# automl/TransformersCanDoBayesianInference

Measured on AMD Instinct MI355X. Metric: synthetic datasets/sec (GP prior, bptt=2000), higher is better.
Workload: dtype fp16; 1 GPU; priors.fast_gp, bptt=2000, num_features=18, emsize=512, nhead=4, nhid=1024, nlayers=6, 1000 bars (BASELINE.json configs[1]); per_gpu_batch=64, global_batch=64, aggregate_k_gradients=1, aggregate_streams=0, aggregate_stacked=False, seq_len=2000, parallelism=dp1, micro_batch_streams=2, eval_pos=weighted sampler(2000)

## Files before the change

transformerscandobayesianinference_amd/csrc/gemm_tn.hip:

```cpp
#include <type_traits>
#include "pfn_device.h"
#include "pfn_kernels.h"

namespace pfn {

PFN_DEV int xcd_remap(int bid, int nwg) {
  const int q = nwg >> 3, r = nwg & 7, xcd = bid & 7;
  return (xcd < r ? xcd * (q + 1) : r * (q + 1) + (xcd - r) * q) + (bid >> 3);
}
typedef __attribute__((address_space(1))) const void gvoid_t;
typedef __attribute__((address_space(3))) void lvoid_t;

constexpr int TN_BMK = 32;

template <typename T>
__global__ __launch_bounds__(256, 2) void gemm_tn_kernel(GemmTN g) {
  constexpr int RB = 128 * sizeof(T);
  constexpr int TILE = TN_BMK * RB;
  extern __shared__ __attribute__((aligned(16))) char smem_raw[];
  LdsPtr smem = lds_cast(smem_raw);
  auto tileA = [&](int buf) { return smem + buf * 2 * TILE; };
  auto tileB = [&](int buf) { return smem + buf * 2 * TILE + TILE; };

  const int p0 = blockIdx.y * 128, q0 = blockIdx.x * 128;
// ... 30 lines not shown
      if constexpr (sizeof(T) == 2) {
        const X8<T> v = __builtin_bit_cast(X8<T>, sa.regs[i]);
#pragma unroll
        for (int e = 0; e < 8; ++e) csum[e] += (float)v[e];
      } else {
        const f32x4 v = __builtin_bit_cast(f32x4, sa.regs[i]);
#pragma unroll
        for (int e = 0; e < 4; ++e) csum[e] += v[e];
      }
    }
  };
  sa.issue(A, g.lda, rows_total, colsA);
  sb.issue(B, g.ldb, rows_total, colsB);
  add_colsum();
  sa.template commit<true>(tileA(0));
  sb.template commit<true>(tileB(0));
  __syncthreads();
  for (int t = 0; t < nt; ++t) {
    const int cur = t & 1;
    if (t + 1 < nt) {
      const long r1 = (long)(t + 1) * TN_BMK;
      sa.issue(A + r1 * g.lda, g.lda, rows_total - (int)r1, colsA);
      sb.issue(B + r1 * g.ldb, g.ldb, rows_total - (int)r1, colsB);
      add_colsum();
    }
    const lds_char* ta = tileA(cur);
    const lds_char* tb = tileB(cur);
#pragma unroll
    for (int ks = 0; ks < TN_BMK; ks += 16) {
      Frag<T> fa[2], fb[2];
#pragma unroll
      for (int i = 0; i < 2; ++i) fa[i] = load_frag_tr<T, RB, 1>(ta, ks, wp * 64 + i * 32);
#pragma unroll
      for (int j = 0; j < 2; ++j) fb[j] = load_frag_tr<T, RB, 1>(tb, ks, wq * 64 + j * 32);
#pragma unroll
      for (int i = 0; i < 2; ++i)
#pragma unroll
        for (int j = 0; j < 2; ++j) acc[i][j] = mma32(fa[i], fb[j], acc[i][j]);
    }
    if (t + 1 < nt) {
      sa.template commit<true>(tileA(cur ^ 1));
      sb.template commit<true>(tileB(cur ^ 1));
    }
    __syncthreads();
  }

  const float osc = loss_scale_down(g.scale_amax);
  if (do_colsum) {
    constexpr int NCH = RB / 16;
    float* red = reinterpret_cast<float*>(smem_raw);
#pragma unroll
    for (int e = 0; e < EPC; ++e) red[threadIdx.x * EPC + e] = csum[e];
    __syncthreads();
    if (threadIdx.x < NCH) {
#pragma unroll
      for (int e = 0; e < EPC; ++e) {
        float t = 0.f;
        for (int j = 0; j < 256 / NCH; ++j) t += red[(j * NCH + threadIdx.x) * EPC + e];
        const int col = p0 + threadIdx.x * EPC + e;
        if (col < g.P) unsafeAtomicAdd(g.colsum + col, t * loss_scale_down(g.scale_amax));
      }
    }
  }
#pragma unroll
  for (int i = 0; i < 2; ++i)
#pragma unroll
    for (int j = 0; j < 2; ++j)
#pragma unroll
      for (int r = 0; r < 16; ++r) {
        const int p = p0 + wp * 64 + i * 32 + acc_row(r, lane);
        const int q = q0 + wq * 64 + j * 32 + (lane & 31);
        if (p < g.P && q < g.Q) {
          float* c = g.C + (long)p * g.ldc + q;
          if (g.atomic) unsafeAtomicAdd(c, acc[i][j][r] * osc);
          else *c = acc[i][j][r] * osc;
        }
      }
}

#ifndef PFN_TNB_KT
#define PFN_TNB_KT 64
#define PFN_TNB_NS 2
#endif
constexpr int TNB_KT = PFN_TNB_KT;
constexpr int TNB_NS = PFN_TNB_NS;
constexpr int TNB_TILE = TNB_KT * 512;
constexpr int TNB_PW = TNB_KT / 16;
constexpr int TNB_LDS = TNB_NS * 2 * TNB_TILE;
static_assert(TNB_LDS <= 160 * 1024 && TNB_KT % 16 == 0 && TNB_NS >= 2 && (TNB_NS - 2) * 2 * TNB_PW < 64, "weight-gradient ring does not fit");

template <typename T>
__global__ __launch_bounds__(512, 1) void gemm_tn_big_kernel(GemmTNGroup g) {
  extern __shared__ __attribute__((aligned(16))) char smem_raw[];
  LdsPtr smem = lds_cast(smem_raw);

  const int ntiles = g.tile_start[g.n];
  const int id = xcd_remap(blockIdx.x, ntiles * g.splits);
  const int split = id / ntiles, tile = id % ntiles;
  int pi = 0;
  while (tile >= g.tile_start[pi + 1]) ++pi;
  const TnProblem& pr = g.p[pi];
  const int tq = pr.Q / 256;
  const int tl = tile - g.tile_start[pi];
  const int p0 = (tl / tq) * 256, q0 = (tl % tq) * 256;
  const long mbeg = (long)split * g.m_chunk;
  const long mend = min((long)g.M, mbeg + g.m_chunk);
  const int rows_total = (int)(mend - mbeg);
  if (rows_total <= 0) return;

  const int wave = __builtin_amdgcn_readfirstlane(threadIdx.x >> 6), lane = threadIdx.x & 63;
  const int wp = wave >> 2, wq = wave & 3;

  const T* pa[TNB_PW];
  const T* pb[TNB_PW];
  int prow[TNB_PW];
#pragma unroll
  for (int i = 0; i < TNB_PW; ++i) {
    const int row = (wave + 8 * i) * 2 + (lane >> 5);
    const int unit = ((lane & 31) >> 2) ^ (row & 3);
    const int col = unit * 32 + (lane & 3) * 8;
    prow[i] = row;
    pa[i] = reinterpret_cast<const T*>(pr.A) + mbeg * pr.lda + p0 + col;
    pb[i] = reinterpret_cast<const T*>(pr.B) + mbeg * pr.ldb + q0 + col;
  }
  auto stage = [&](int slot, int r0) {
    LdsPtr ta = smem + slot * 2 * TNB_TILE + wave * 1024;
    LdsPtr tb = ta + TNB_TILE;
#pragma unroll
    for (int i = 0; i < TNB_PW; ++i) {
      const long r = min(r0 + prow[i], rows_total - 1) & g.debug_mask;
      dma16_global(pa[i] + r * pr.lda, ta + i * 8192);
      dma16_global(pb[i] + r * pr.ldb, tb + i * 8192);
    }
  };

  f32x16 acc[4][2];
#pragma unroll
  for (int i = 0; i < 4; ++i)
#pragma unroll
    for (int j = 0; j < 2; ++j)
#pragma unroll
      for (int r = 0; r < 16; ++r) acc[i][j][r] = 0.f;
  f32x16 cs;
#pragma unroll
  for (int r = 0; r < 16; ++r) cs[r] = 0.f;
  const bool do_colsum = pr.colsum != nullptr && q0 == 0;
  Frag<T> ones;
#pragma unroll
  for (int e = 0; e < 8; ++e) ones.v[e] = (T)1.0f;

  const int nt = (rows_total + TNB_KT - 1) / TNB_KT;
#pragma unroll
  for (int st = 0; st < TNB_NS - 1; ++st)
    if (st < nt) stage(st, st * TNB_KT);
  auto wait_stage = [&](int younger) {
    switch (younger) {
      case 0: wait_vm_barrier<0>(); break;
      case 1: wait_vm_barrier<(TNB_NS > 2 ? 1 : 0) * 2 * TNB_PW>(); break;
      case 2: wait_vm_barrier<(TNB_NS > 3 ? 2 : 0) * 2 * TNB_PW>(); break;
      case 3: wait_vm_barrier<(TNB_NS > 4 ? 3 : 0) * 2 * TNB_PW>(); break;
      default: wait_vm_barrier<(TNB_NS - 2) * 2 * TNB_PW>(); break;
    }
  };
  static_assert(TNB_NS <= 6, "wait_stage cases");
  auto main_loop = [&](auto with_colsum) {
    constexpr bool CS = decltype(with_colsum)::value;
    int slot = 0, slot_next = TNB_NS - 1;
    for (int t = 0; t < nt; ++t) {
      wait_stage(min(nt - t - 1, TNB_NS - 2));
      if (t + TNB_NS - 1 < nt) stage(slot_next, (t + TNB_NS - 1) * TNB_KT);
      LdsPtr ta = smem + slot * 2 * TNB_TILE;
      LdsPtr tb = ta + TNB_TILE;
      const int valid = rows_total - t * TNB_KT;
      if (valid < TNB_KT) {
        for (int idx = threadIdx.x; idx < (TNB_KT - valid) * 32; idx += 512) {
          const u32x4 z = {0u, 0u, 0u, 0u};
          lds_write16(ta + (valid + idx / 32) * 512 + (idx % 32) * 16, z);
        }
        __syncthreads();
      }
#pragma unroll
      for (int ks = 0; ks < TNB_KT; ks += 16) {
        Frag<T> fa[4], fb[2];
#pragma unroll
        for (int j = 0; j < 2; ++j) fb[j] = load_frag_tr<T, 512, 1>(tb, ks, wq * 64 + j * 32);
#pragma unroll
        for (int i = 0; i < 4; ++i) fa[i] = load_frag_tr<T, 512, 1>(ta, ks, wp * 128 + i * 32);
#pragma unroll
        for (int i = 0; i < 4; ++i)
#pragma unroll
          for (int j = 0; j < 2; ++j) acc[i][j] = mma32(fa[i], fb[j], acc[i][j]);
        if constexpr (CS) cs = mma32(load_frag_tr<T, 512, 1>(ta, ks, wp * 128 + wq * 32), ones, cs);
      }
      slot_next = slot;
      slot = slot + 1 == TNB_NS ? 0 : slot + 1;
    }
  };
  if (do_colsum) main_loop(std::true_type{});
  else main_loop(std::false_type{});

  const int pv = pr.Pv > 0 ? pr.Pv : pr.P;
  const float osc = loss_scale_down(g.scale_amax);
  if (do_colsum && (lane & 31) == 0) {
#pragma unroll
    for (int r = 0; r < 16; ++r) {
      const int pp = p0 + wp * 128 + wq * 32 + acc_row(r, lane);
      if (pp < pv) unsafeAtomicAdd(pr.colsum + pp, cs[r] * osc);
    }
  }
  const bool atomic = true;
#pragma unroll
  for (int i = 0; i < 4; ++i)
#pragma unroll
    for (int j = 0; j < 2; ++j)
#pragma unroll
      for (int r = 0; r < 16; ++r) {
        const int pp = p0 + wp * 128 + i * 32 + acc_row(r, lane);
        const int qq = q0 + wq * 64 + j * 32 + (lane & 31);
        float* c = pr.C + (long)pp * pr.ldc + qq;
        if (pp >= pv) continue;
        if (atomic) unsafeAtomicAdd(c, acc[i][j][r] * osc);
        else *c += acc[i][j][r] * osc;
      }
}

constexpr int TNW_NW = 4;
constexpr int TNW_PW = TNB_KT / 2 / TNW_NW;
static_assert(TNB_KT == 64 && TNB_NS == 2, "gemm_tn_wide_kernel is written for two 64-token stages");
template <typename T>
__global__ __launch_bounds__(TNW_NW * 64, 1) void gemm_tn_wide_kernel(GemmTNGroup g) {
  extern __shared__ __attribute__((aligned(16))) char smem_raw[];
  LdsPtr smem = lds_cast(smem_raw);
  const int ntiles = g.tile_start[g.n];
  const int id = xcd_remap(blockIdx.x, ntiles * g.splits);
  const int split = id / ntiles, tile = id % ntiles;
  int pi = 0;
  while (tile >= g.tile_start[pi + 1]) ++pi;
  const TnProblem& pr = g.p[pi];
  const int tq = pr.Q / 256;
  const int tl = tile - g.tile_start[pi];
  const int p0 = (tl / tq) * 256, q0 = (tl % tq) * 256;
  const long mbeg = (long)split * g.m_chunk;
  const long mend = min((long)g.M, mbeg + g.m_chunk);
  const int rows_total = (int)(mend - mbeg);
  if (rows_total <= 0) return;
  const int wave = __builtin_amdgcn_readfirstlane(threadIdx.x >> 6), lane = threadIdx.x & 63;
  const int wp = wave >> 1, wq = wave & 1;

  const int prow0 = wave * 2 + (lane >> 5);
  const int pcol = ((((lane & 31) >> 2) ^ (prow0 & 3)) * 32) + (lane & 3) * 8;
  const T* pa = reinterpret_cast<const T*>(pr.A) + mbeg * pr.lda + p0 + pcol;
  const T* pb = reinterpret_cast<const T*>(pr.B) + mbeg * pr.ldb + q0 + pcol;
  const long lda = pr.lda, ldb = pr.ldb;
  auto stage = [&](int slot, int r0) {
    LdsPtr ta = smem + slot * 2 * TNB_TILE + wave * 1024;
    LdsPtr tb = ta + TNB_TILE;
#pragma unroll
    for (int i = 0; i < TNW_PW; ++i) {
      const long r = min(r0 + prow0 + 2 * TNW_NW * i, rows_total - 1) & g.debug_mask;
      dma16_global(pa + r * lda, ta + i * TNW_NW * 1024);
      dma16_global(pb + r * ldb, tb + i * TNW_NW * 1024);
    }
  };

  f32x16 acc[4][4];
#pragma unroll
  for (int i = 0; i < 4; ++i)
#pragma unroll
    for (int j = 0; j < 4; ++j)
#pragma unroll
      for (int r = 0; r < 16; ++r) acc[i][j][r] = 0.f;
  float cs[2] = {0.f, 0.f};
  const bool do_colsum = pr.colsum != nullptr && q0 == 0;

  const int nt = (rows_total + TNB_KT - 1) / TNB_KT;
  struct Frs { Frag<T> a[4], b[4]; };
  auto main_loop = [&](auto with_colsum) {
    constexpr bool CS = decltype(with_colsum)::value;
    Frs f0, f1;
    auto ld = [&](Frs& f, const lds_char* ta, const lds_char* tb, int ks) {
#pragma unroll
      for (int j = 0; j < 4; ++j) f.b[j] = load_frag_tr<T, 512, 1>(tb, ks, wq * 128 + j * 32);
#pragma unroll
      for (int i = 0; i < 4; ++i) f.a[i] = load_frag_tr<T, 512, 1>(ta, ks, wp * 128 + i * 32);
    };
    auto mm = [&](const Frs& f) {
#pragma unroll
      for (int i = 0; i < 4; ++i)
#pragma unroll
        for (int j = 0; j < 4; ++j) acc[i][j] = mma32(f.a[i], f.b[j], acc[i][j]);
      if constexpr (CS) {
#pragma unroll
        for (int c = 0; c < 2; ++c)
#pragma unroll
          for (int e = 0; e < 8; ++e) cs[c] += (float)(wq ? f.a[2 + c] : f.a[c]).v[e];
      }
    };
    auto enter_stage = [&](int t, int slot) {
      wait_vm_barrier<0>();
      if (t + 1 < nt) stage(slot ^ 1, (t + 1) * TNB_KT);
      const int valid = rows_total - t * TNB_KT;
      if (valid < TNB_KT) {
        LdsPtr ta = smem + slot * 2 * TNB_TILE;
        for (int idx = threadIdx.x; idx < (TNB_KT - valid) * 32; idx += TNW_NW * 64) {
          const u32x4 z = {0u, 0u, 0u, 0u};
          lds_write16(ta + (valid + idx / 32) * 512 + (idx % 32) * 16, z);
        }
        __syncthreads();
      }
    };
    int slot = 0;
    enter_stage(0, slot);
    ld(f0, smem, smem + TNB_TILE, 0);
    for (int t = 0; t < nt; ++t) {
      const lds_char* ta = smem + slot * 2 * TNB_TILE;
      const lds_char* tb = ta + TNB_TILE;
      ld(f1, ta, tb, 16);
      PFN_PIN_LDS_MFMA();
      mm(f0);
      PFN_PIN_LDS_MFMA();
      ld(f0, ta, tb, 32);
      PFN_PIN_LDS_MFMA();
      mm(f1);
      PFN_PIN_LDS_MFMA();
      ld(f1, ta, tb, 48);
      PFN_PIN_LDS_MFMA();
      mm(f0);
      PFN_PIN_LDS_MFMA();
      slot ^= 1;
      if (t + 1 < nt) {
        enter_stage(t + 1, slot);
        const lds_char* tan = smem + slot * 2 * TNB_TILE;
        ld(f0, tan, tan + TNB_TILE, 0);
      }
      PFN_PIN_LDS_MFMA();
      mm(f1);
      PFN_PIN_LDS_MFMA();
    }
  };
  stage(0, 0);
  if (do_colsum) main_loop(std::true_type{});
  else main_loop(std::false_type{});

  const int pv = pr.Pv > 0 ? pr.Pv : pr.P;
  const float osc = loss_scale_down(g.scale_amax);
  if (do_colsum) {
#pragma unroll
    for (int c = 0; c < 2; ++c) {
      const float s = cs[c] + __shfl_xor(cs[c], 32, 64);
      const int pp = p0 + wp * 128 + (2 * wq + c) * 32 + (lane & 31);
      if (lane < 32 && pp < pv) unsafeAtomicAdd(pr.colsum + pp, s * osc);
    }
  }
#pragma unroll
  for (int i = 0; i < 4; ++i)
#pragma unroll
    for (int j = 0; j < 4; ++j)
#pragma unroll
      for (int r = 0; r < 16; ++r) {
        const int pp = p0 + wp * 128 + i * 32 + acc_row(r, lane);
        const int qq = q0 + wq * 128 + j * 32 + (lane & 31);
        if (pp < pv) unsafeAtomicAdd(pr.C + (long)pp * pr.ldc + qq, acc[i][j][r] * osc);
      }
}

static bool aligned16(const void* p) { return (reinterpret_cast<uintptr_t>(p) & 15) == 0; }

static int g_tn_debug_wrap = 0;
void set_gemm_tn_debug_wrap(int rows) { g_tn_debug_wrap = rows; }
static int g_tn_group_splits = 0;
void set_gemm_tn_group_splits(int splits) { g_tn_group_splits = splits; }
static bool g_tn_wide = false;
void set_gemm_tn_group_waves(int waves) { g_tn_wide = waves == 4; }

int launch_gemm_tn(GemmTN g, int precision, hipStream_t stream) {
  if (g.M <= 0 || g.P <= 0 || g.Q <= 0) return PFN_OK;
  const size_t es = prec_esize(precision);
  if ((g.lda * es) % 16 || (g.ldb * es) % 16 || !aligned16(g.A) || !aligned16(g.B)) return PFN_ERR_ALIGNMENT;
  const int tp = (g.P + 127) / 128, tq = (g.Q + 127) / 128;
  int splits = (1024 + tp * tq - 1) / (tp * tq);
  const int max_splits = (g.M + 4 * TN_BMK - 1) / (4 * TN_BMK);
  if (splits > max_splits) splits = max_splits;
  if (g.max_splits > 0 && splits > g.max_splits) splits = g.max_splits;
  if (splits < 1) splits = 1;
  if (!g.atomic) splits = 1;
  int chunk = (g.M + splits - 1) / splits;
  chunk = (chunk + TN_BMK - 1) / TN_BMK * TN_BMK;
  splits = (g.M + chunk - 1) / chunk;
  g.m_chunk = chunk;
  const size_t lds = 4 * TN_BMK * 128 * es;
  PFN_DISPATCH_OP(precision, hipLaunchKernelGGL(gemm_tn_kernel<T>, dim3(tq, tp, splits), dim3(256), lds, stream, g));
  return hipGetLastError() == hipSuccess ? PFN_OK : PFN_ERR_LAUNCH;
}

bool gemm_tn_group_supported(const TnProblem& p) {
  return p.P % 256 == 0 && p.Q % 256 == 0 && (p.lda * 2) % 16 == 0 && (p.ldb * 2) % 16 == 0 && aligned16(p.A) && aligned16(p.B);
}

int launch_gemm_tn_group(GemmTNGroup g, int precision, hipStream_t stream) {
  if (g.n <= 0 || g.M <= 0) return PFN_OK;
  if (g.n > TN_GROUP_MAX) return PFN_ERR_ARGUMENT;
  if (!prec_is16(precision)) return PFN_ERR_UNSUPPORTED;
  int tiles = 0;
  for (int i = 0; i < g.n; ++i) {
    if (!gemm_tn_group_supported(g.p[i])) return PFN_ERR_UNSUPPORTED;
    g.tile_start[i] = tiles;
    tiles += (g.p[i].P / 256) * (g.p[i].Q / 256);
  }
  g.tile_start[g.n] = tiles;
  int splits = g.splits;
  if (splits <= 0 && g_tn_group_splits > 0) splits = g_tn_group_splits;
  if (splits <= 0) {
    splits = 8;
    for (int sp = 1; sp <= 8; ++sp) {
      const int blocks = tiles * sp, rounds = (blocks + 255) / 256;
      if (blocks >= 0.9 * rounds * 256) { splits = sp; break; }
    }
  }
  const int max_splits = (g.M + 4 * TNB_KT - 1) / (4 * TNB_KT);
  if (splits > max_splits) splits = max_splits;
  int chunk = (g.M + splits - 1) / splits;
  chunk = (chunk + TNB_KT - 1) / TNB_KT * TNB_KT;
  splits = (g.M + chunk - 1) / chunk;
  g.splits = splits;
  g.m_chunk = chunk;
  g.debug_mask = g_tn_debug_wrap > 0 ? g_tn_debug_wrap - 1 : 0x7fffffff;
  if (g_tn_wide) {
    static LdsAllowance allow_w[2];
    if (precision == PFN_PREC_FP16) {
      allow_w[1].ensure(gemm_tn_wide_kernel<f16>, TNB_LDS);
      hipLaunchKernelGGL(gemm_tn_wide_kernel<f16>, dim3(tiles * splits), dim3(TNW_NW * 64), TNB_LDS, stream, g);
    } else {
      allow_w[0].ensure(gemm_tn_wide_kernel<bf16>, TNB_LDS);
      hipLaunchKernelGGL(gemm_tn_wide_kernel<bf16>, dim3(tiles * splits), dim3(TNW_NW * 64), TNB_LDS, stream, g);
    }
    return hipGetLastError() == hipSuccess ? PFN_OK : PFN_ERR_LAUNCH;
  }
  static LdsAllowance allowance[2];
  if (precision == PFN_PREC_FP16) {
    allowance[1].ensure(gemm_tn_big_kernel<f16>, TNB_LDS);
    hipLaunchKernelGGL(gemm_tn_big_kernel<f16>, dim3(tiles * splits), dim3(512), TNB_LDS, stream, g);
  } else {
    allowance[0].ensure(gemm_tn_big_kernel<bf16>, TNB_LDS);
    hipLaunchKernelGGL(gemm_tn_big_kernel<bf16>, dim3(tiles * splits), dim3(512), TNB_LDS, stream, g);
  }
  return hipGetLastError() == hipSuccess ? PFN_OK : PFN_ERR_LAUNCH;
}

}
```

transformerscandobayesianinference_amd/csrc/pfn_api.hip:

```cpp
#include <algorithm>
#include <cstdarg>
#include <cstdio>
#include <cstring>
#include <mutex>
#include <vector>
#include "pfn_kernels.h"

using namespace pfn;

namespace pfn {
namespace {
struct ProfPair { hipEvent_t a, b; };
std::mutex g_prof_mu;
std::vector<ProfPair> g_prof[PFN_PROF_SLOTS];
std::atomic<int> g_prof_on{0};
}
bool prof_enabled() { return g_prof_on.load(std::memory_order_relaxed) != 0; }
void* prof_begin(int slot, hipStream_t s) {
  const int on = g_prof_on.load(std::memory_order_relaxed);
  if (!on || slot < 0 || slot >= PFN_PROF_SLOTS) return nullptr;
  if (on >= 2 && (slot & ~1) != on - 2) return nullptr;
  ProfPair* p = new ProfPair;
  if (hipEventCreate(&p->a) != hipSuccess || hipEventCreate(&p->b) != hipSuccess) { delete p; return nullptr; }
  (void)hipEventRecord(p->a, s);
// ... 300 lines not shown
  const pfn_model_desc& d = *m.d;
  const int prec = d.precision, E = d.emsize, F = d.nhid;
  const float* params = m.params;
  hipStream_t s = m.s;
  const bool y16u = pl.y16u;
  if (pl.fuse_ln) {
    ProfScope ps(PFN_PROF_GEMM_OUT_LN + prof, s);
    GemmLN g; memset(&g, 0, sizeof(g));
    g.A = u.ctx; g.lda = E; g.B = W(m, p.w_o); g.ldb = E; g.M = rows; g.N = E; g.K = E; g.bias = params + p.b_o;
    set_resid(g, res);
    g.gamma = params + p.g1; g.beta = params + p.be1; g.eps = d.ln_eps;
    g.y = u.y1; g.mean = u.mean1; g.rstd = u.rstd1; g.x_t = u.x1_t; g.y16 = pl.y16;
    PFN_TRY(launch_gemm_ln(g, prec, s));
    res = Resid{nullptr, u.y1, u.mean1, u.rstd1, params + p.g1, params + p.be1};
  } else {
    {
      GemmNT g = nt(u.ctx, E, W(m, p.w_o), E, rows, E, E, EPI_BIAS | (pdrop > 0.f ? 0 : EPI_RESID) | EPI_OUT_F32);
      g.bias = params + p.b_o; g.resid = u.xin; g.ld_resid = E; g.out_f32 = u.y1; g.ld_out_f32 = E;
      if (y16u) { g.flags = EPI_BIAS | EPI_RESID_T | EPI_OUT_T; g.aux = u.xin_t; g.ld_aux = E; g.out_t = u.y1; g.ld_out_t = E; }
      PFN_TRY(launch_gemm_nt(g, prec, s));
      if (pdrop > 0.f) PFN_TRY(launch_dropout_add(u.y1, u.xin, rows, E, seed[1], pdrop, s));
    }
    PFN_TRY(launch_layernorm_fwd(u.y1, params + p.g1, params + p.be1, y16u ? nullptr : u.x1, u.x1_t, u.mean1, u.rstd1, rows, E, d.ln_eps, prec, s, y16u));
  }
  {
    ProfScope ps(PFN_PROF_GEMM_LIN1 + prof, s);
    GemmNT g = nt(u.x1_t, E, W(m, p.w1), E, rows, F, E, EPI_BIAS | EPI_GELU | EPI_OUT_T | EPI_OUT2_T);
    g.bias = params + p.b1; g.out_t = u.h; g.ld_out_t = F; g.out2_t = u.hpre; g.ld_out2 = F;
    PFN_TRY(launch_gemm_nt(g, prec, s));
    if (pdrop > 0.f) PFN_TRY(launch_dropout_scale(u.h, u.h, u.hpre, u.hpre, rows, F, seed[2], pdrop, prec, s));
  }
  if (pl.fuse_ln) {
    ProfScope ps(PFN_PROF_GEMM_LIN2_LN + prof, s);
    GemmLN g; memset(&g, 0, sizeof(g));
    g.A = u.h; g.lda = F; g.B = W(m, p.w2); g.ldb = F; g.M = rows; g.N = E; g.K = F; g.bias = params + p.b2;
    set_resid(g, res);
    g.gamma = params + p.g2; g.beta = params + p.be2; g.eps = d.ln_eps;
    g.y = u.y2; g.mean = u.mean2; g.rstd = u.rstd2; g.x_t = u.x2_t; g.y16 = pl.y16;
    g.x_f32 = last ? u.x2 : nullptr;
    PFN_TRY(launch_gemm_ln(g, prec, s));
    res = Resid{nullptr, u.y2, u.mean2, u.rstd2, params + p.g2, params + p.be2};
  } else {
    {
      GemmNT g = nt(u.h, F, W(m, p.w2), F, rows, E, F, EPI_BIAS | (pdrop > 0.f ? 0 : EPI_RESID) | EPI_OUT_F32);
      g.bias = params + p.b2; g.resid = u.x1; g.ld_resid = E; g.out_f32 = u.y2; g.ld_out_f32 = E;
      if (y16u) { g.flags = EPI_BIAS | EPI_RESID_T | EPI_OUT_T; g.aux = u.x1_t; g.ld_aux = E; g.out_t = u.y2; g.ld_out_t = E; }
      PFN_TRY(launch_gemm_nt(g, prec, s));
      if (pdrop > 0.f) PFN_TRY(launch_dropout_add(u.y2, u.x1, rows, E, seed[3], pdrop, s));
    }
    PFN_TRY(launch_layernorm_fwd(u.y2, params + p.g2, params + p.be2, (y16u && !last) ? nullptr : u.x2, u.x2_t, u.mean2, u.rstd2, rows, E, d.ln_eps, prec, s, y16u));
  }
  return PFN_OK;
}

int decoder_forward(const Model& m, const void* xt_t, char* dt, char* dpre, float* logits, int rows) {
  const int prec = m.d->precision, E = m.d->emsize, F = m.d->nhid, O = m.d->n_out;
  {
    GemmNT g = nt(xt_t, E, W(m, m.L->dec0_w), E, rows, F, E, EPI_BIAS | EPI_GELU | EPI_OUT_T | EPI_OUT2_T);
    g.bias = m.params + m.L->dec0_b; g.out_t = dt; g.ld_out_t = F; g.out2_t = dpre; g.ld_out2 = F;
    PFN_TRY(launch_gemm_nt(g, prec, m.s));
  }
  GemmNT g = nt(dt, F, W(m, m.L->dec2_w), F, rows, O, F, EPI_BIAS | EPI_OUT_F32);
  g.bias = m.params + m.L->dec2_b; g.out_f32 = logits; g.ld_out_f32 = O;
  return launch_gemm_nt(g, prec, m.s);
}
int decoder_backward_data(const Model& m, const void* dlog_t, const void* dpre, char* dd_t, float* dxt, int rows) {
  const int prec = m.d->precision, E = m.d->emsize, F = m.d->nhid, O = m.d->n_out, npad = m.L->n_out_pad;
  {
    GemmNT g = nt(dlog_t, npad, WT(m, m.L->dec2_wt), npad, rows, F, npad % 64 == 0 ? npad : O, EPI_GELU_BWD | EPI_OUT_T);
    g.aux = dpre; g.ld_aux = F; g.out_t = dd_t; g.ld_out_t = F;
    PFN_TRY(launch_gemm_nt(g, prec, m.s));
  }
  GemmNT g = nt(dd_t, F, WT(m, m.L->dec0_wt), F, rows, E, F, EPI_OUT_F32);
  g.out_f32 = dxt; g.ld_out_f32 = E;
  return launch_gemm_nt(g, prec, m.s);
}

bool tn_set_groupable(const std::vector<TnProblem>& probs, int prec) {
  bool grouped = prec_is16(prec);
  for (const TnProblem& t : probs) grouped = grouped && gemm_tn_group_supported(t);
  return grouped;
}
int launch_tn_set(const std::vector<TnProblem>& probs, int rows, int prec, bool det, const float* lsc, int prof_slot, hipStream_t s, bool allow_group = true) {
  if (!(allow_group && tn_set_groupable(probs, prec))) {
    for (const TnProblem& t : probs) {
      GemmTN g = tn(t.A, t.lda, t.B, t.ldb, t.C, t.ldc, rows, t.Pv ? t.Pv : t.P, t.Q, t.colsum);
      if (det) g.max_splits = 1;
      g.scale_amax = lsc;
      PFN_TRY(launch_gemm_tn(g, prec, s));
    }
    return PFN_OK;
  }
  for (size_t i0 = 0; i0 < probs.size(); i0 += TN_GROUP_MAX) {
    ProfScope ps(prof_slot, s);
    GemmTNGroup g;
    memset(&g, 0, sizeof(g));
    g.n = (int)std::min<size_t>(TN_GROUP_MAX, probs.size() - i0);
    g.M = rows;
    g.splits = det ? 1 : 0;
    g.scale_amax = lsc;
    for (int i = 0; i < g.n; ++i) g.p[i] = probs[i0 + i];
    PFN_TRY(launch_gemm_tn_group(g, prec, s));
  }
  return PFN_OK;
}

struct LnSinks { float *dgamma, *dbeta, *dbias; };
struct LayerGrads {
  const void* dout; int dout_is_t;
  const void* y2; const float *mean2, *rstd2, *gamma2; const void* y1; const float *mean1, *rstd1, *gamma1; const void* hpre;
  char *dy2_t, *dy2m_t, *dh_t, *dy1_t, *dqkv_t, *dx1_t;
  LnSinks ln2, ln1;
  float* ln_part;
};
GemmLNB lnb(const Model& m, const Plan& pl, const float* lsc, const void* A, long lda, const void* Bw, long ldb, int K, const void* aux, const void* y,
            const float* mean, const float* rstd, const float* gamma, void* dx_t, const LnSinks& sink, int rows) {
  GemmLNB g; memset(&g, 0, sizeof(g));
  g.A = A; g.lda = lda; g.B = Bw; g.ldb = ldb; g.M = rows; g.N = m.d->emsize; g.K = K; g.aux = aux;
  g.y = y; g.mean = mean; g.rstd = rstd; g.gamma = gamma; g.dx_t = dx_t; g.dgamma = sink.dgamma; g.dbeta = sink.dbeta; g.scale_amax = lsc; g.y16 = pl.y16_any;
  return g;
}
GemmLNB lnb_dy1(const Model& m, const Plan& pl, const float* lsc, const LayerP& t, const LayerGrads& g, int rows) {
  const int F = m.d->nhid;
  return lnb(m, pl, lsc, g.dh_t, F, WT(m, t.w1), F, F, g.dy2_t, g.y1, g.mean1, g.rstd1, g.gamma1, g.dy1_t, g.ln1, rows);
}
GemmLNB lnb_dx(const Model& m, const Plan& pl, const float* lsc, const LayerP& t, const char* dqkv_t, const char* dy1_t, const LayerGrads& below, int rows) {
  const int E = m.d->emsize;
  return lnb(m, pl, lsc, dqkv_t, 3 * E, WT(m, t.w_in), 3 * E, 3 * E, dy1_t, below.y2, below.mean2, below.rstd2, below.gamma2, below.dy2_t, below.ln2, rows);
}
bool lnbwd_fusable(const Model& m, const Plan& pl, const float* lsc, const LayerGrads& g0, int rows) {
  const LayerP& t = m.L->layer_t[0];
  return pl.lnb_eligible && gemm_lnbwd_supported(lnb_dy1(m, pl, lsc, t, g0, rows)) && gemm_lnbwd_supported(lnb_dx(m, pl, lsc, t, g0.dqkv_t, g0.dy1_t, g0, rows));
}
int layer_backward_to_dy1(const Model& m, const LayerP& t, const LayerGrads& g, int rows, const Plan& pl, bool fuse_lnb, bool ln2_done, const float* lsc,
                          float pdrop, unsigned seed2, int prof) {
  const int prec = m.d->precision, E = m.d->emsize, F = m.d->nhid;
  hipStream_t s = m.s;
  if (!ln2_done)
    PFN_TRY(launch_layernorm_bwd(g.dout, g.dout_is_t, g.y2, g.gamma2, g.mean2, g.rstd2, nullptr, g.dy2_t, g.ln2.dgamma, g.ln2.dbeta, g.ln2.dbias, rows, E, prec, s,
                                 g.ln_part, lsc, pl.y16_any));
  const char* dy2_op = g.dy2_t;
  if (pdrop > 0.f) { PFN_TRY(launch_dropout_scale(g.dy2_t, g.dy2m_t, nullptr, nullptr, rows, E, seed2, pdrop, prec, s)); dy2_op = g.dy2m_t; }
  {
    ProfScope ps(PFN_PROF_GEMM_DHPRE + prof, s);
    GemmNT gm = nt(dy2_op, E, WT(m, t.w2), E, rows, F, E, EPI_GELU_BWD | EPI_OUT_T);
    gm.aux = g.hpre; gm.ld_aux = F; gm.out_t = g.dh_t; gm.ld_out_t = F;
    PFN_TRY(launch_gemm_nt(gm, prec, s));
  }
  if (fuse_lnb) {
    ProfScope ps(PFN_PROF_GEMM_DY1 + prof, s);
    PFN_TRY(launch_gemm_lnbwd(lnb_dy1(m, pl, lsc, t, g, rows), prec, s));
  } else {
    {
      GemmNT gm = nt(g.dh_t, F, WT(m, t.w1), F, rows, E, F, EPI_RESID_T | EPI_OUT_T);
      gm.aux = g.dy2_t; gm.ld_aux = E; gm.out_t = g.dx1_t; gm.ld_out_t = E;
      PFN_TRY(launch_gemm_nt(gm, prec, s));
    }
    PFN_TRY(launch_layernorm_bwd(g.dx1_t, 1, g.y1, g.gamma1, g.mean1, g.rstd1, nullptr, g.dy1_t, g.ln1.dgamma, g.ln1.dbeta, g.ln1.dbias, rows, E, prec, s,
                                 g.ln_part, lsc, pl.y16_any));
  }
  return PFN_OK;
}
int layer_backward_dx(const Model& m, const LayerP& t, const char* dqkv_t, const char* dy1_t, int rows, const Plan& pl, const float* lsc, const LayerGrads* below,
                      float* gA, char* gA_t, bool out_f32, int prof) {
  const int prec = m.d->precision, E = m.d->emsize;
  if (below) {
    ProfScope ps(PFN_PROF_GEMM_DX + prof, m.s);
    return launch_gemm_lnbwd(lnb_dx(m, pl, lsc, t, dqkv_t, dy1_t, *below, rows), prec, m.s);
  }
  GemmNT g = nt(dqkv_t, 3 * E, WT(m, t.w_in), 3 * E, rows, E, 3 * E, EPI_RESID_T | (out_f32 ? EPI_OUT_F32 : EPI_OUT_T));
  g.aux = dy1_t; g.ld_aux = E; g.out_f32 = gA; g.ld_out_f32 = E; g.out_t = gA_t; g.ld_out_t = E;
  return launch_gemm_nt(g, prec, m.s);
}

}

extern "C" {

static bool g_gp_planes = true;
static bool g_fuse_delta = true;
static int g_default_schedule = 0;
static bool top_layer_on_test_rows(const pfn_model_desc& d, int S, int sep, float pdrop) {
  return !(d.schedule & PFN_SCHED_TOP_LAYER_ALL_ROWS) && d.nlayers > 0 && pdrop == 0.f && d.dropout == 0.f && sep < S && 4L * sep >= S;
}
static bool top_layer_on_test_rows_ragged(const pfn_model_desc& d, int S, const Ragged& rg, float pdrop) {
// ... 1028 lines not shown
```

transformerscandobayesianinference_amd/csrc/pfn_device.h:

```cpp
#pragma once
#include <hip/hip_runtime.h>
#include <stdint.h>

namespace pfn {

typedef __bf16 bf16;
typedef __attribute__((ext_vector_type(8))) __bf16 bf16x8;
typedef __attribute__((ext_vector_type(4))) __bf16 bf16x4;
typedef __attribute__((ext_vector_type(2))) __bf16 bf16x2;
typedef _Float16 f16;
typedef __attribute__((ext_vector_type(8))) _Float16 f16x8;
typedef __attribute__((ext_vector_type(4))) _Float16 f16x4;
typedef __attribute__((ext_vector_type(2))) _Float16 f16x2;
typedef __attribute__((ext_vector_type(16))) float f32x16;
typedef __attribute__((ext_vector_type(4))) float f32x4;
typedef __attribute__((ext_vector_type(2))) float f32x2;
typedef __attribute__((ext_vector_type(4))) unsigned int u32x4;
typedef __attribute__((ext_vector_type(2))) unsigned int u32x2;
template <typename T> struct OpVec;
template <> struct OpVec<bf16> { typedef bf16x8 x8; typedef bf16x4 x4; typedef bf16x2 x2; };
template <> struct OpVec<f16> { typedef f16x8 x8; typedef f16x4 x4; typedef f16x2 x2; };
template <> struct OpVec<float> { typedef f32x4 x8; typedef f32x4 x4; typedef f32x2 x2; };
template <typename T> using X8 = typename OpVec<T>::x8;
template <typename T> using X4 = typename OpVec<T>::x4;
// ... 151 lines not shown
    const int colb = (col0 + 16 * g + 4 * (i & 3)) * 2;
    const int ra = (MAP == 1) ? (k0 + 8 * h) : (k0 + 4 * h);
    const int rb = (MAP == 1) ? (k0 + 8 * h + 4) : (k0 + 8 + 4 * h);
    const auto lo = ds_read_tr16_b64<T>(tile + (ra + (i >> 2)) * STRIDE + colb);
    const auto hi = ds_read_tr16_b64<T>(tile + (rb + (i >> 2)) * STRIDE + colb);
    f.v = __builtin_shufflevector(lo, hi, 0, 1, 2, 3, 4, 5, 6, 7);
  } else {
    const int colb = (col0 + (l & 31)) * 4;
#pragma unroll
    for (int e = 0; e < 8; ++e) {
      const int row = (MAP == 1) ? (k0 + 8 * h + e) : (k0 + 8 * (e >> 2) + 4 * h + (e & 3));
      f.v[e] = lds_read_f32(tile + row * STRIDE + colb);
    }
  }
  return f;
}

template <typename T> PFN_DEV void store_row_block(T* row_block, const float (&v)[16], int h, bool valid) {
  if constexpr (sizeof(T) == 2) {
#pragma unroll
    for (int p = 0; p < 2; ++p) {
      typedef typename OpVec<T>::x2 x2;
      x2 a0 = {(T)v[8 * p + 0], (T)v[8 * p + 1]}, a1 = {(T)v[8 * p + 2], (T)v[8 * p + 3]};
      x2 b0 = {(T)v[8 * p + 4], (T)v[8 * p + 5]}, b1 = {(T)v[8 * p + 6], (T)v[8 * p + 7]};
      const auto r0 = __builtin_amdgcn_permlane32_swap(__builtin_bit_cast(unsigned, a0), __builtin_bit_cast(unsigned, b0), false, false);
      const auto r1 = __builtin_amdgcn_permlane32_swap(__builtin_bit_cast(unsigned, a1), __builtin_bit_cast(unsigned, b1), false, false);
      const u32x4 w = {r0[0], r1[0], r0[1], r1[1]};
      if (valid) *reinterpret_cast<u32x4*>(row_block + 16 * p + 8 * h) = w;
    }
  } else {
#pragma unroll
    for (int rg = 0; rg < 4; ++rg)
      if (valid) *reinterpret_cast<f32x4*>(row_block + 8 * rg + 4 * h) = f32x4{v[4 * rg], v[4 * rg + 1], v[4 * rg + 2], v[4 * rg + 3]};
  }
}

template <typename T> PFN_DEV void store_frag_pair_blocked(T* block, const Frag<T>& f0, const Frag<T>& f1, int j, int h, bool valid) {
  char* base = reinterpret_cast<char*>(block);
  if constexpr (sizeof(T) == 2) {
#pragma unroll
    for (int p = 0; p < 2; ++p) {
      const u32x4 d = __builtin_bit_cast(u32x4, p == 0 ? f0.v : f1.v);
      const auto r0 = __builtin_amdgcn_permlane32_swap(d[0], d[2], false, false);
      const auto r1 = __builtin_amdgcn_permlane32_swap(d[1], d[3], false, false);
      const u32x4 w = {r0[0], r1[0], r0[1], r1[1]};
      if (valid) __builtin_nontemporal_store(w, reinterpret_cast<u32x4*>(base + ((p * 32 + j) * 2 + h) * 16));
    }
  } else {
#pragma unroll
    for (int p = 0; p < 2; ++p) {
      const Frag<T>& f = p == 0 ? f0 : f1;
#pragma unroll
      for (int sub = 0; sub < 2; ++sub)
        if (valid) __builtin_nontemporal_store(f32x4{f.v[4 * sub], f.v[4 * sub + 1], f.v[4 * sub + 2], f.v[4 * sub + 3]},
                                               reinterpret_cast<f32x4*>(base + (((2 * p + sub) * 32 + j) * 2 + h) * 16));
    }
  }
}
template <typename T> PFN_DEV int blocked_chunk_row(int w) { return (w >> 1) & 31; }
template <typename T> PFN_DEV int blocked_chunk_col(int w) {
  if constexpr (sizeof(T) == 2) return 16 * (w >> 6) + 8 * (w & 1);
  else return 8 * (w >> 6) + 4 * (w & 1);
}

typedef __amdgpu_buffer_rsrc_t BufRsrc;
PFN_DEV BufRsrc make_rsrc(const void* base, long bytes) {
  const int n = bytes > 0x7ffffff0L ? 0x7ffffff0 : (bytes < 0 ? 0 : (int)bytes);
  return __builtin_amdgcn_make_buffer_rsrc(const_cast<void*>(base), 0, n, 0x00020000);
}
PFN_DEV u32x4 buf_load16(BufRsrc r, int byte_offset) { return __builtin_amdgcn_raw_buffer_load_b128(r, byte_offset, 0, 0); }
constexpr int BUF_OOB = 0x7ffffff0;

struct DmaRsrc { u32x4 w; };
PFN_DEV DmaRsrc make_dma_rsrc(const void* base, long bytes) {
  const unsigned long long p = (unsigned long long)base;
  const int n = bytes > 0x7ffffff0L ? 0x7ffffff0 : (bytes < 0 ? 0 : (int)bytes);
  DmaRsrc r;
  r.w[0] = __builtin_amdgcn_readfirstlane((unsigned)p);
  r.w[1] = __builtin_amdgcn_readfirstlane((unsigned)(p >> 32) & 0xffffu);
  r.w[2] = __builtin_amdgcn_readfirstlane((unsigned)n);
  r.w[3] = 0x00020000u;
  return r;
}
PFN_DEV void dma16(const DmaRsrc& r, LdsPtr lds_dst_uniform, int byte_offset) {
  unsigned keep;
  const unsigned dst = __builtin_amdgcn_readfirstlane((unsigned)(unsigned long long)lds_dst_uniform);
  const u32x4 w = {(unsigned)__builtin_amdgcn_readfirstlane(r.w[0]), (unsigned)__builtin_amdgcn_readfirstlane(r.w[1]),
                   (unsigned)__builtin_amdgcn_readfirstlane(r.w[2]), (unsigned)__builtin_amdgcn_readfirstlane(r.w[3])};
  asm volatile("s_mov_b32 %0, m0\n\ts_mov_b32 m0, %1\n\ts_nop 0\n\tbuffer_load_dwordx4 %2, %3, 0 offen lds\n\ts_mov_b32 m0, %0"
               : "=&s"(keep) : "s"(dst), "v"(byte_offset), "s"(w) : "memory");
}
PFN_DEV void dma4(const DmaRsrc& r, LdsPtr lds_dst_uniform, int byte_offset) {
  unsigned keep;
  const unsigned dst = __builtin_amdgcn_readfirstlane((unsigned)(unsigned long long)lds_dst_uniform);
  const u32x4 w = {(unsigned)__builtin_amdgcn_readfirstlane(r.w[0]), (unsigned)__builtin_amdgcn_readfirstlane(r.w[1]),
                   (unsigned)__builtin_amdgcn_readfirstlane(r.w[2]), (unsigned)__builtin_amdgcn_readfirstlane(r.w[3])};
  asm volatile("s_mov_b32 %0, m0\n\ts_mov_b32 m0, %1\n\ts_nop 0\n\tbuffer_load_dword %2, %3, 0 offen lds\n\ts_mov_b32 m0, %0"
               : "=&s"(keep) : "s"(dst), "v"(byte_offset), "s"(w) : "memory");
}
PFN_DEV void dma16_global(const void* src, LdsPtr lds_dst_uniform) {
  unsigned keep;
  const unsigned dst = __builtin_amdgcn_readfirstlane((unsigned)(unsigned long long)lds_dst_uniform);
  asm volatile("s_mov_b32 %0, m0\n\ts_mov_b32 m0, %1\n\ts_nop 0\n\tglobal_load_lds_dwordx4 %2, off\n\ts_mov_b32 m0, %0"
               : "=&s"(keep) : "s"(dst), "v"(src) : "memory");
}
template <int N> PFN_DEV void wait_vm_barrier() {
  __builtin_amdgcn_s_waitcnt(0x0070 | (N & 15) | ((N >> 4) << 14));
  asm volatile("s_waitcnt vmcnt(%0) lgkmcnt(0)\n\ts_barrier" :: "n"(N) : "memory");
}
PFN_DEV void dma_wait_all() {
  __builtin_amdgcn_s_waitcnt(0x0F70);
  asm volatile("s_waitcnt vmcnt(0)" ::: "memory");
}

template <typename T, int ROWS, int RB, int NT> struct TileStageBuf {
  static constexpr int NCH = RB / 16;
  static constexpr int TOTAL = ROWS * NCH;
  static constexpr int PER = (TOTAL + NT - 1) / NT;
  u32x4 regs[PER];
  int voff[PER];
  PFN_DEV void init(int ld_bytes) {
#pragma unroll
    for (int i = 0; i < PER; ++i) {
      const int id = threadIdx.x + i * NT;
      voff[i] = (TOTAL % NT == 0 || id < TOTAL) ? (id / NCH) * ld_bytes + (id % NCH) * 16 : BUF_OOB;
    }
  }
  PFN_DEV void issue(BufRsrc r, int tile_byte_offset) {
#pragma unroll
    for (int i = 0; i < PER; ++i) regs[i] = buf_load16(r, voff[i] + tile_byte_offset);
  }
  template <int STRIDE> PFN_DEV void commit_p(LdsPtr tile) const {
#pragma unroll
    for (int i = 0; i < PER; ++i) {
      const int id = threadIdx.x + i * NT;
      if (TOTAL % NT != 0 && id >= TOTAL) break;
      lds_write16(tile + (id / NCH) * STRIDE + (id % NCH) * 16, regs[i]);
    }
  }
};

template <typename T, int ROWS, int RB, int NT> struct TileStage {
  static constexpr int NCH = RB / 16;
  static constexpr int TOTAL = ROWS * NCH;
  static constexpr int PER = (TOTAL + NT - 1) / NT;
  static constexpr int EPC = 16 / sizeof(T);
  u32x4 regs[PER];

  PFN_DEV void issue(const T* src, long ld, int rows_valid, int cols_valid) {
#pragma unroll
    for (int i = 0; i < PER; ++i) {
      const int id = threadIdx.x + i * NT;
      const int row = id / NCH, c = id % NCH;
      u32x4 v = {0u, 0u, 0u, 0u};
      if ((TOTAL % NT == 0 || id < TOTAL) && row < rows_valid && (c + 1) * EPC <= cols_valid)
        v = *reinterpret_cast<const u32x4*>(src + (long)row * ld + c * EPC);
      else if ((TOTAL % NT == 0 || id < TOTAL) && row < rows_valid && c * EPC < cols_valid) {
        T tmp[EPC];
#pragma unroll
        for (int e = 0; e < EPC; ++e) tmp[e] = (c * EPC + e < cols_valid) ? src[(long)row * ld + c * EPC + e] : (T)0.f;
        v = *reinterpret_cast<u32x4*>(tmp);
      }
      regs[i] = v;
    }
  }
  template <int STRIDE> PFN_DEV void commit_p(LdsPtr tile) const {
// ... 103 lines not shown
```

Measured before the change: 2513 datasets/s.

## Stage weight-gradient GEMM tiles via buffer-resource DMA with late issue after first MFMA

Replaces per-row global-pointer DMA staging in the TN weight-gradient kernels with a buffer-resource stager that advances a base address per K tile. Out-of-range rows are now zero-filled by the hardware bounds check, so the LDS zero-fill pass and its extra barrier go away. In the big kernel the next stage's loads are issued after the first MFMA sub-step instead of before compute, so address math and issue overlap with matrix work. The cost is a host-side support check with a per-problem fallback when strides or split sizes exceed the buffer range, and the simple two-stage wait assumes the default ring depth.

After: 2548 datasets/s (median of 6 runs). +1.4%, better.

```diff
diff --git a/transformerscandobayesianinference_amd/csrc/gemm_tn.hip b/transformerscandobayesianinference_amd/csrc/gemm_tn.hip
--- a/transformerscandobayesianinference_amd/csrc/gemm_tn.hip
+++ b/transformerscandobayesianinference_amd/csrc/gemm_tn.hip
@@ -136,12 +136,54 @@
 #define PFN_TNB_KT 64
 #define PFN_TNB_NS 2
 #endif
+#ifndef PFN_TNB_LATE_ISSUE
+#define PFN_TNB_LATE_ISSUE 1
+#endif
 constexpr int TNB_KT = PFN_TNB_KT;
 constexpr int TNB_NS = PFN_TNB_NS;
 constexpr int TNB_TILE = TNB_KT * 512;
 constexpr int TNB_PW = TNB_KT / 16;
 constexpr int TNB_LDS = TNB_NS * 2 * TNB_TILE;
 static_assert(TNB_LDS <= 160 * 1024 && TNB_KT % 16 == 0 && TNB_NS >= 2 && (TNB_NS - 2) * 2 * TNB_PW < 64, "weight-gradient ring does not fit");
+constexpr long TN_GROUP_MAX_SPLIT_BYTES = 0x7ffffff0L;
+
+template <int NW> struct TnStager {
+  static constexpr int NP = TNB_KT / 2 / NW;
+  DmaRsrc ra, rb;
+  unsigned a_lo, a_hi, b_lo, b_hi;
+  unsigned step_a, step_b;
+  int va[NP], vb[NP];
+  int wave, srow, mask;
+  PFN_DEV void init(const TnProblem& pr, long mbeg, int rows, int p0, int q0, int wave_, int lane, int debug_mask) {
+    const long lda2 = pr.lda * 2, ldb2 = pr.ldb * 2;
+    ra = make_dma_rsrc(reinterpret_cast<const char*>(pr.A) + mbeg * lda2 + p0 * 2, (rows - 1) * lda2 + 512);
+    rb = make_dma_rsrc(reinterpret_cast<const char*>(pr.B) + mbeg * ldb2 + q0 * 2, (rows - 1) * ldb2 + 512);
+    a_lo = ra.w[0]; a_hi = ra.w[1]; b_lo = rb.w[0]; b_hi = rb.w[1];
+    step_a = __builtin_amdgcn_readfirstlane((unsigned)(TNB_KT * lda2));
+    step_b = __builtin_amdgcn_readfirstlane((unsigned)(TNB_KT * ldb2));
+    wave = wave_; srow = 0; mask = debug_mask;
+    const int row0 = wave * 2 + (lane >> 5);
+    const int colb = ((((lane & 31) >> 2) ^ (row0 & 3)) * 32 + (lane & 3) * 8) * 2;
+#pragma unroll
+    for (int i = 0; i < NP; ++i) {
+      va[i] = (row0 + 2 * NW * i) * (int)lda2 + colb;
+      vb[i] = (row0 + 2 * NW * i) * (int)ldb2 + colb;
+    }
+  }
+  PFN_DEV void issue(LdsPtr slot) {
+    LdsPtr ta = slot + wave * 1024;
+    LdsPtr tb = ta + TNB_TILE;
+#pragma unroll
+    for (int i = 0; i < NP; ++i) {
+      dma16(ra, ta + i * NW * 1024, va[i]);
+      dma16(rb, tb + i * NW * 1024, vb[i]);
+    }
+    dma_rsrc_advance(ra, step_a);
+    dma_rsrc_advance(rb, step_b);
+    srow += TNB_KT;
+    if ((srow & mask) == 0) { ra.w[0] = a_lo; ra.w[1] = a_hi; rb.w[0] = b_lo; rb.w[1] = b_hi; }
+  }
+};
 
 template <typename T>
 __global__ __launch_bounds__(512, 1) void gemm_tn_big_kernel(GemmTNGroup g) {
@@ -165,28 +207,9 @@
   const int wave = __builtin_amdgcn_readfirstlane(threadIdx.x >> 6), lane = threadIdx.x & 63;
   const int wp = wave >> 2, wq = wave & 3;
 
-  const T* pa[TNB_PW];
-  const T* pb[TNB_PW];
-  int prow[TNB_PW];
-#pragma unroll
-  for (int i = 0; i < TNB_PW; ++i) {
-    const int row = (wave + 8 * i) * 2 + (lane >> 5);
-    const int unit = ((lane & 31) >> 2) ^ (row & 3);
-    const int col = unit * 32 + (lane & 3) * 8;
-    prow[i] = row;
-    pa[i] = reinterpret_cast<const T*>(pr.A) + mbeg * pr.lda + p0 + col;
-    pb[i] = reinterpret_cast<const T*>(pr.B) + mbeg * pr.ldb + q0 + col;
-  }
-  auto stage = [&](int slot, int r0) {
-    LdsPtr ta = smem + slot * 2 * TNB_TILE + wave * 1024;
-    LdsPtr tb = ta + TNB_TILE;
-#pragma unroll
-    for (int i = 0; i < TNB_PW; ++i) {
-      const long r = min(r0 + prow[i], rows_total - 1) & g.debug_mask;
-      dma16_global(pa[i] + r * pr.lda, ta + i * 8192);
-      dma16_global(pb[i] + r * pr.ldb, tb + i * 8192);
-    }
-  };
+  TnStager<8> stg;
+  stg.init(pr, mbeg, rows_total, p0, q0, wave, lane, g.debug_mask);
+  static_assert(TnStager<8>::NP == TNB_PW, "wait_stage counts 2 TNB_PW DMA instructions per stage");
 
   f32x16 acc[4][2];
 #pragma unroll
@@ -206,8 +229,9 @@
   const int nt = (rows_total + TNB_KT - 1) / TNB_KT;
 #pragma unroll
   for (int st = 0; st < TNB_NS - 1; ++st)
-    if (st < nt) stage(st, st * TNB_KT);
+    if (st < nt) stg.issue(smem + st * 2 * TNB_TILE);
   auto wait_stage = [&](int younger) {
+    if constexpr (TNB_NS == 2) { wait_vm_barrier<0>(); return; }
     switch (younger) {
       case 0: wait_vm_barrier<0>(); break;
       case 1: wait_vm_barrier<(TNB_NS > 2 ? 1 : 0) * 2 * TNB_PW>(); break;
@@ -222,17 +246,10 @@
     int slot = 0, slot_next = TNB_NS - 1;
     for (int t = 0; t < nt; ++t) {
       wait_stage(min(nt - t - 1, TNB_NS - 2));
-      if (t + TNB_NS - 1 < nt) stage(slot_next, (t + TNB_NS - 1) * TNB_KT);
+      const bool more = t + TNB_NS - 1 < nt;
+      if (!PFN_TNB_LATE_ISSUE && more) stg.issue(smem + slot_next * 2 * TNB_TILE);
       LdsPtr ta = smem + slot * 2 * TNB_TILE;
       LdsPtr tb = ta + TNB_TILE;
-      const int valid = rows_total - t * TNB_KT;
-      if (valid < TNB_KT) {
-        for (int idx = threadIdx.x; idx < (TNB_KT - valid) * 32; idx += 512) {
-          const u32x4 z = {0u, 0u, 0u, 0u};
-          lds_write16(ta + (valid + idx / 32) * 512 + (idx % 32) * 16, z);
-        }
-        __syncthreads();
-      }
 #pragma unroll
       for (int ks = 0; ks < TNB_KT; ks += 16) {
         Frag<T> fa[4], fb[2];
@@ -245,6 +262,11 @@
 #pragma unroll
           for (int j = 0; j < 2; ++j) acc[i][j] = mma32(fa[i], fb[j], acc[i][j]);
         if constexpr (CS) cs = mma32(load_frag_tr<T, 512, 1>(ta, ks, wp * 128 + wq * 32), ones, cs);
+        if (PFN_TNB_LATE_ISSUE && ks == 0) {
+          PFN_PIN_LDS_MFMA();
+          if (more) stg.issue(smem + slot_next * 2 * TNB_TILE);
+          PFN_PIN_LDS_MFMA();
+        }
       }
       slot_next = slot;
       slot = slot + 1 == TNB_NS ? 0 : slot + 1;
@@ -278,9 +300,9 @@
       }
 }
 
+#define PFN_TNW_BUILT (PFN_TNB_KT == 64 && PFN_TNB_NS == 2)
+#if PFN_TNW_BUILT
 constexpr int TNW_NW = 4;
-constexpr int TNW_PW = TNB_KT / 2 / TNW_NW;
-static_assert(TNB_KT == 64 && TNB_NS == 2, "gemm_tn_wide_kernel is written for two 64-token stages");
 template <typename T>
 __global__ __launch_bounds__(TNW_NW * 64, 1) void gemm_tn_wide_kernel(GemmTNGroup g) {
   extern __shared__ __attribute__((aligned(16))) char smem_raw[];
@@ -301,21 +323,8 @@
   const int wave = __builtin_amdgcn_readfirstlane(threadIdx.x >> 6), lane = threadIdx.x & 63;
   const int wp = wave >> 1, wq = wave & 1;
 
-  const int prow0 = wave * 2 + (lane >> 5);
-  const int pcol = ((((lane & 31) >> 2) ^ (prow0 & 3)) * 32) + (lane & 3) * 8;
-  const T* pa = reinterpret_cast<const T*>(pr.A) + mbeg * pr.lda + p0 + pcol;
-  const T* pb = reinterpret_cast<const T*>(pr.B) + mbeg * pr.ldb + q0 + pcol;
-  const long lda = pr.lda, ldb = pr.ldb;
-  auto stage = [&](int slot, int r0) {
-    LdsPtr ta = smem + slot * 2 * TNB_TILE + wave * 1024;
-    LdsPtr tb = ta + TNB_TILE;
-#pragma unroll
-    for (int i = 0; i < TNW_PW; ++i) {
-      const long r = min(r0 + prow0 + 2 * TNW_NW * i, rows_total - 1) & g.debug_mask;
-      dma16_global(pa + r * lda, ta + i * TNW_NW * 1024);
-      dma16_global(pb + r * ldb, tb + i * TNW_NW * 1024);
-    }
-  };
+  TnStager<TNW_NW> stg;
+  stg.init(pr, mbeg, rows_total, p0, q0, wave, lane, g.debug_mask);
 
   f32x16 acc[4][4];
 #pragma unroll
@@ -352,16 +361,7 @@
     };
     auto enter_stage = [&](int t, int slot) {
       wait_vm_barrier<0>();
-      if (t + 1 < nt) stage(slot ^ 1, (t + 1) * TNB_KT);
-      const int valid = rows_total - t * TNB_KT;
-      if (valid < TNB_KT) {
-        LdsPtr ta = smem + slot * 2 * TNB_TILE;
-        for (int idx = threadIdx.x; idx < (TNB_KT - valid) * 32; idx += TNW_NW * 64) {
-          const u32x4 z = {0u, 0u, 0u, 0u};
-          lds_write16(ta + (valid + idx / 32) * 512 + (idx % 32) * 16, z);
-        }
-        __syncthreads();
-      }
+      if (t + 1 < nt) stg.issue(smem + (slot ^ 1) * 2 * TNB_TILE);
     };
     int slot = 0;
     enter_stage(0, slot);
@@ -392,7 +392,7 @@
       PFN_PIN_LDS_MFMA();
     }
   };
-  stage(0, 0);
+  stg.issue(smem);
   if (do_colsum) main_loop(std::true_type{});
   else main_loop(std::false_type{});
 
@@ -417,6 +417,7 @@
         if (pp < pv) unsafeAtomicAdd(pr.C + (long)pp * pr.ldc + qq, acc[i][j][r] * osc);
       }
 }
+#endif
 
 static bool aligned16(const void* p) { return (reinterpret_cast<uintptr_t>(p) & 15) == 0; }
 
@@ -478,8 +479,14 @@
   splits = (g.M + chunk - 1) / chunk;
   g.splits = splits;
   g.m_chunk = chunk;
-  g.debug_mask = g_tn_debug_wrap > 0 ? g_tn_debug_wrap - 1 : 0x7fffffff;
+  for (int i = 0; i < g.n; ++i) {
+    const TnProblem& p = g.p[i];
+    if (p.lda < 256 || p.ldb < 256 || (long)chunk * p.lda * 2 > TN_GROUP_MAX_SPLIT_BYTES || (long)chunk * p.ldb * 2 > TN_GROUP_MAX_SPLIT_BYTES) return PFN_ERR_UNSUPPORTED;
+  }
+  const int wrap = g_tn_debug_wrap;
+  g.debug_mask = wrap >= TNB_KT && (wrap & (wrap - 1)) == 0 ? wrap - 1 : 0x7fffffff;
   if (g_tn_wide) {
+#if PFN_TNW_BUILT
     static LdsAllowance allow_w[2];
     if (precision == PFN_PREC_FP16) {
       allow_w[1].ensure(gemm_tn_wide_kernel<f16>, TNB_LDS);
@@ -489,6 +496,9 @@
       hipLaunchKernelGGL(gemm_tn_wide_kernel<bf16>, dim3(tiles * splits), dim3(TNW_NW * 64), TNB_LDS, stream, g);
     }
     return hipGetLastError() == hipSuccess ? PFN_OK : PFN_ERR_LAUNCH;
+#else
+    return PFN_ERR_UNSUPPORTED;
+#endif
   }
   static LdsAllowance allowance[2];
   if (precision == PFN_PREC_FP16) {
diff --git a/transformerscandobayesianinference_amd/csrc/pfn_api.hip b/transformerscandobayesianinference_amd/csrc/pfn_api.hip
--- a/transformerscandobayesianinference_amd/csrc/pfn_api.hip
+++ b/transformerscandobayesianinference_amd/csrc/pfn_api.hip
@@ -406,15 +406,17 @@
   return grouped;
 }
 int launch_tn_set(const std::vector<TnProblem>& probs, int rows, int prec, bool det, const float* lsc, int prof_slot, hipStream_t s, bool allow_group = true) {
-  if (!(allow_group && tn_set_groupable(probs, prec))) {
-    for (const TnProblem& t : probs) {
+  auto one_by_one = [&](size_t i0, size_t n) {
+    for (size_t i = i0; i < i0 + n; ++i) {
+      const TnProblem& t = probs[i];
       GemmTN g = tn(t.A, t.lda, t.B, t.ldb, t.C, t.ldc, rows, t.Pv ? t.Pv : t.P, t.Q, t.colsum);
       if (det) g.max_splits = 1;
       g.scale_amax = lsc;
       PFN_TRY(launch_gemm_tn(g, prec, s));
     }
-    return PFN_OK;
-  }
+    return (int)PFN_OK;
+  };
+  if (!(allow_group && tn_set_groupable(probs, prec))) return one_by_one(0, probs.size());
   for (size_t i0 = 0; i0 < probs.size(); i0 += TN_GROUP_MAX) {
     ProfScope ps(prof_slot, s);
     GemmTNGroup g;
@@ -424,7 +426,9 @@
     g.splits = det ? 1 : 0;
     g.scale_amax = lsc;
     for (int i = 0; i < g.n; ++i) g.p[i] = probs[i0 + i];
-    PFN_TRY(launch_gemm_tn_group(g, prec, s));
+    const int rc = launch_gemm_tn_group(g, prec, s);
+    if (rc == PFN_ERR_UNSUPPORTED) PFN_TRY(one_by_one(i0, g.n));
+    else PFN_TRY(rc);
   }
   return PFN_OK;
 }
diff --git a/transformerscandobayesianinference_amd/csrc/pfn_device.h b/transformerscandobayesianinference_amd/csrc/pfn_device.h
--- a/transformerscandobayesianinference_amd/csrc/pfn_device.h
+++ b/transformerscandobayesianinference_amd/csrc/pfn_device.h
@@ -257,6 +257,12 @@
   r.w[3] = 0x00020000u;
   return r;
 }
+PFN_DEV void dma_rsrc_advance(DmaRsrc& r, unsigned bytes) {
+  const unsigned long long b = (((unsigned long long)r.w[1] << 32) | r.w[0]) + bytes;
+  r.w[0] = (unsigned)b;
+  r.w[1] = (unsigned)(b >> 32);
+  r.w[2] = (unsigned)max((int)r.w[2] - (int)bytes, 0);
+}
 PFN_DEV void dma16(const DmaRsrc& r, LdsPtr lds_dst_uniform, int byte_offset) {
   unsigned keep;
   const unsigned dst = __builtin_amdgcn_readfirstlane((unsigned)(unsigned long long)lds_dst_uniform);
```
